# anihcsam/OpenGaussian

Measured on AMD Instinct MI355X. Metric: fwd+bwd Mpix/s at 1080p, 1M Gaussians (RGB+6-D ins_feat); k-means it/s, higher is better.
Workload: dtype f32; 1 GPU; S1M-1080p RGB(SH3)+depth+alpha (all grads) + 6-ch ins_feat (grad to ins_feat) fwd+bwd, ONE fused 9-channel pass; gaussians=1000000, width=1920, height=1080, views_cycled=8, parallelism=single

## Files before the change

opengaussian_amd/csrc/binning.hip:

```cpp
#include <stdlib.h>
#include <string.h>

#include "ogs_common.h"

namespace ogs {

namespace {

constexpr size_t kSweepHeaderWords = 4 * 256 + 4 + 60;
constexpr int kScanItems = 8;
constexpr int kScanTile = kBlock * kScanItems;

__device__ __forceinline__ uint32_t wave_inclusive_scan(uint32_t v) {
#pragma unroll
    for (int d = 1; d < kWave; d <<= 1) {
        uint32_t t = __shfl_up(v, d, kWave);
        if (lane_id() >= d) v += t;
    }
    return v;
}

__device__ __forceinline__ uint32_t block_exclusive_scan(uint32_t v, uint32_t& total, uint32_t* wave_sums ) {
    const int wave = threadIdx.x >> 6;
    const uint32_t inc = wave_inclusive_scan(v);
    if (lane_id() == kWave - 1) wave_sums[wave] = inc;
    __syncthreads();
    uint32_t base = 0, tot = 0;
#pragma unroll
    for (int w = 0; w < kBlock / kWave; ++w) {
        const uint32_t s = wave_sums[w];
        if (w < wave) base += s;
        tot += s;
    }
    total = tot;
    __syncthreads();
    return base + inc - v;
}

__device__ __forceinline__ void load_items(const uint32_t* __restrict__ in, const uint32_t* __restrict__ gather,
                                           int64_t base, int64_t n, uint32_t item[kScanItems]) {
#pragma unroll
    for (int i = 0; i < kScanItems; ++i) {
        const int64_t idx = base + i;
        uint32_t v = 0;
        if (idx < n) v = gather ? in[gather[idx]] : in[idx];
        item[i] = v;
    }
}

__global__ __launch_bounds__(kBlock) void scan_reduce_kernel(const uint32_t* __restrict__ in,
                                                             const uint32_t* __restrict__ gather, int64_t n,
                                                             uint32_t* __restrict__ partials, const uint32_t* __restrict__ n_dev) {
    __shared__ uint32_t wave_sums[4];
    if (n_dev) n = min(n, (int64_t)*n_dev);
    const int64_t base = (int64_t)blockIdx.x * kScanTile + (int64_t)threadIdx.x * kScanItems;
    uint32_t item[kScanItems];
    load_items(in, gather, base, n, item);
    uint32_t s = 0;
#pragma unroll
    for (int i = 0; i < kScanItems; ++i) s += item[i];
    uint32_t total;
    block_exclusive_scan(s, total, wave_sums);
    if (threadIdx.x == 0) partials[blockIdx.x] = total;
}

template <bool SUM_PARTIALS>
__global__ __launch_bounds__(kBlock) void scan_apply_kernel(const uint32_t* __restrict__ in,
                                                            const uint32_t* __restrict__ gather,
                                                            uint32_t* __restrict__ out, int64_t n,
                                                            const uint32_t* __restrict__ partial_offsets,
                                                            uint32_t* __restrict__ total_out, const uint32_t* __restrict__ n_dev) {
    __shared__ uint32_t wave_sums[4];
    if (n_dev) n = min(n, (int64_t)*n_dev);
    const int64_t base = (int64_t)blockIdx.x * kScanTile + (int64_t)threadIdx.x * kScanItems;
    uint32_t item[kScanItems];
    load_items(in, gather, base, n, item);
    uint32_t s = 0;
#pragma unroll
    for (int i = 0; i < kScanItems; ++i) s += item[i];
    uint32_t block_base = 0;
    if (SUM_PARTIALS) {
        uint32_t acc = 0;
        for (uint32_t j = threadIdx.x; j < blockIdx.x; j += kBlock) acc += partial_offsets[j];
        uint32_t tot;
        block_exclusive_scan(acc, tot, wave_sums);
        block_base = tot;
    } else if (partial_offsets) {
        block_base = partial_offsets[blockIdx.x];
    }
    uint32_t total;
    uint32_t run = block_exclusive_scan(s, total, wave_sums) + block_base;
#pragma unroll
    for (int i = 0; i < kScanItems; ++i) {
        const int64_t idx = base + i;
        if (idx < n) out[idx] = run;
        run += item[i];
    }
    if (total_out && threadIdx.x == 0) {
        if (SUM_PARTIALS) { if (blockIdx.x == gridDim.x - 1) *total_out = block_base + total; }
        else if (partial_offsets == nullptr) *total_out = total;
    }
}

__global__ void scan_total_kernel(const uint32_t* __restrict__ in, const uint32_t* __restrict__ gather,
                                  const uint32_t* __restrict__ out, int64_t n, uint32_t* __restrict__ total_out,
                                  const uint32_t* __restrict__ n_dev) {
    if (threadIdx.x == 0 && blockIdx.x == 0) {
        if (n_dev) n = min(n, (int64_t)*n_dev);
        if (n <= 0) { *total_out = 0u; return; }
        const uint32_t last = gather ? in[gather[n - 1]] : in[n - 1];
        *total_out = out[n - 1] + last;
    }
}

inline int scan_blocks(int64_t n) { return (int)((n + kScanTile - 1) / kScanTile); }
constexpr int kFlatScanBlocks = 16384;

template <int ITEMS>
__global__ __launch_bounds__(kBlock) void radix_hist_kernel(const uint32_t* __restrict__ keys, int64_t n_cap,
                                                            const uint32_t* __restrict__ n_dev, int shift,
                                                            int bits, uint32_t* __restrict__ hist, int nblocks, bool drop) {
    __shared__ uint32_t h[256];
    const int64_t n = n_dev ? min((int64_t)*n_dev, n_cap) : n_cap;
    const int ndig = 1 << bits;
    const uint32_t mask = ndig - 1;
    h[threadIdx.x] = 0;
    __syncthreads();
    const int64_t base = (int64_t)blockIdx.x * (kBlock * ITEMS);
#pragma unroll
    for (int i = 0; i < ITEMS; ++i) {
        const int64_t idx = base + i * kBlock + threadIdx.x;
        if (idx < n) {
            const uint32_t k = keys[idx];
            if (!(drop && k == kDropKey)) atomicAdd(&h[(k >> shift) & mask], 1u);
        }
    }
    __syncthreads();
    if ((int)threadIdx.x < ndig) hist[(size_t)threadIdx.x * nblocks + blockIdx.x] = h[threadIdx.x];
}

__global__ __launch_bounds__(kBlock) void radix_rowscan_kernel(uint32_t* __restrict__ hist, int nblocks,
                                                               uint32_t* __restrict__ row_total) {
    __shared__ uint32_t wave_sums[4];
    uint32_t* row = hist + (size_t)blockIdx.x * nblocks;
    uint32_t carry = 0;
    for (int base = 0; base < nblocks; base += kScanTile) {
        uint32_t item[kScanItems];
        const int b0 = base + (int)threadIdx.x * kScanItems;
        uint32_t sum = 0;
#pragma unroll
        for (int i = 0; i < kScanItems; ++i) {
            item[i] = (b0 + i < nblocks) ? row[b0 + i] : 0u;
            sum += item[i];
        }
        uint32_t total;
        uint32_t run = carry + block_exclusive_scan(sum, total, wave_sums);
#pragma unroll
        for (int i = 0; i < kScanItems; ++i) {
            if (b0 + i < nblocks) row[b0 + i] = run;
            run += item[i];
        }
        carry += total;
    }
    if (threadIdx.x == 0) row_total[blockIdx.x] = carry;
}

template <int ITEMS>
__global__ __launch_bounds__(kBlock) void radix_scatter_kernel(const uint32_t* __restrict__ keys_in,
                                                               const uint32_t* __restrict__ vals_in,
                                                               uint32_t* __restrict__ keys_out,
                                                               uint32_t* __restrict__ vals_out, int64_t n_cap,
                                                               const uint32_t* __restrict__ n_dev, int shift,
                                                               int bits, const uint32_t* __restrict__ offsets,
                                                               const uint32_t* __restrict__ row_total,
                                                               int nblocks, bool drop, uint32_t* __restrict__ kept_out) {
    __shared__ uint32_t wave_hist_s[kBlock / kWave][256];
    __shared__ uint32_t scan_sums[4];
    __shared__ uint32_t dig_start[256], glob_base[256];
    __shared__ uint32_t stage_k[kBlock * ITEMS], stage_v[kBlock * ITEMS];
    volatile uint32_t(*wave_hist)[256] = wave_hist_s;
    const int64_t n = n_dev ? min((int64_t)*n_dev, n_cap) : n_cap;
    const int ndig = 1 << bits;
    const uint32_t mask = ndig - 1;
    const int tid = threadIdx.x, lane = tid & 63, wave = tid >> 6;
#pragma unroll
    for (int w = 0; w < kBlock / kWave; ++w) wave_hist_s[w][tid] = 0;
    __syncthreads();

    const int64_t base = (int64_t)blockIdx.x * (kBlock * ITEMS) + (int64_t)wave * (ITEMS * kWave);
    uint32_t key[ITEMS], val[ITEMS], rank[ITEMS];
#pragma unroll
    for (int i = 0; i < ITEMS; ++i) {
        const int64_t idx = base + i * kWave + lane;
        const bool valid = idx < n;
        key[i] = valid ? keys_in[idx] : 0xFFFFFFFFu;
        val[i] = valid ? vals_in[idx] : 0u;
    }
    const uint64_t lt_mask = (1ull << lane) - 1ull;
#pragma unroll
    for (int i = 0; i < ITEMS; ++i) {
        const int64_t idx = base + i * kWave + lane;
        const bool valid = drop ? key[i] != kDropKey : idx < n;
        const uint32_t d = (key[i] >> shift) & mask;
        uint64_t peers = __ballot(valid);
        for (int b = 0; b < bits; ++b) {
            const bool bit = (d >> b) & 1u;
            const uint64_t m = __ballot(bit);
            peers &= bit ? m : ~m;
        }
        const uint32_t r = __popcll(peers & lt_mask);
        const uint32_t cnt = __popcll(peers);
        uint32_t pre = 0;
        if (valid) pre = wave_hist[wave][d];
        __builtin_amdgcn_wave_barrier();
        if (valid && r == 0) wave_hist[wave][d] = pre + cnt;
        __builtin_amdgcn_wave_barrier();
        rank[i] = pre + r;
    }
    __syncthreads();
    uint32_t run_len = 0;
    if (tid < ndig) {
#pragma unroll
        for (int w = 0; w < kBlock / kWave; ++w) {
            const uint32_t t = wave_hist_s[w][tid];
            wave_hist_s[w][tid] = run_len;
            run_len += t;
        }
    }
    uint32_t n_valid;
    const uint32_t local_start = block_exclusive_scan(run_len, n_valid, scan_sums);
    uint32_t dummy_total;
    const uint32_t digit_base = block_exclusive_scan(tid < ndig ? row_total[tid] : 0u, dummy_total, scan_sums);
    if (kept_out != nullptr && blockIdx.x == 0 && tid == 0) *kept_out = dummy_total;
    if (tid < ndig) {
        dig_start[tid] = local_start;
        glob_base[tid] = digit_base + offsets[(size_t)tid * nblocks + blockIdx.x] - local_start;
    }
    __syncthreads();
#pragma unroll
    for (int i = 0; i < ITEMS; ++i) {
        const int64_t idx = base + i * kWave + lane;
        if (drop ? key[i] != kDropKey : idx < n) {
            const uint32_t d = (key[i] >> shift) & mask;
            const uint32_t lp = dig_start[d] + wave_hist_s[wave][d] + rank[i];
            stage_k[lp] = key[i];
            stage_v[lp] = val[i];
        }
    }
    __syncthreads();
    for (uint32_t j = tid; j < n_valid; j += kBlock) {
        const uint32_t k = stage_k[j];
        const uint32_t pos = glob_base[(k >> shift) & mask] + j;
        keys_out[pos] = k;
        vals_out[pos] = stage_v[j];
    }
}

constexpr uint32_t kStatAgg = 1u << 30, kStatInc = 2u << 30, kStatMask = (1u << 30) - 1u;
constexpr int kSpinLimit = 1 << 22;
constexpr int kLookBack = 8;
constexpr int kHistAllBlocks = 256;

struct RadixPlanDev { int npass; int shift[4]; int bits[4]; };

__global__ __launch_bounds__(kBlock) void radix_hist_all_kernel(const uint32_t* __restrict__ keys, int64_t n_cap,
                                                                const uint32_t* __restrict__ n_dev, RadixPlanDev plan,
                                                                uint32_t* __restrict__ ghist , bool drop) {
    __shared__ uint32_t h[4][256];
    const int64_t n = n_dev ? min((int64_t)*n_dev, n_cap) : n_cap;
#pragma unroll
    for (int p = 0; p < 4; ++p) h[p][threadIdx.x] = 0;
    __syncthreads();
    for (int64_t idx = (int64_t)blockIdx.x * kBlock + threadIdx.x; idx < n; idx += (int64_t)gridDim.x * kBlock) {
        const uint32_t k = keys[idx];
        if (drop && k == kDropKey) continue;
#pragma unroll
        for (int p = 0; p < 4; ++p)
            if (p < plan.npass) atomicAdd(&h[p][(k >> plan.shift[p]) & ((1u << plan.bits[p]) - 1u)], 1u);
    }
    __syncthreads();
#pragma unroll
    for (int p = 0; p < 4; ++p)
        if (p < plan.npass && h[p][threadIdx.x] != 0) atomicAdd(&ghist[p * 256 + threadIdx.x], h[p][threadIdx.x]);
}

template <int ITEMS>
__global__ __launch_bounds__(kBlock) void radix_onesweep_kernel(const uint32_t* __restrict__ keys_in,
                                                                const uint32_t* __restrict__ vals_in,
                                                                uint32_t* __restrict__ keys_out,
                                                                uint32_t* __restrict__ vals_out, int64_t n_cap,
                                                                const uint32_t* __restrict__ n_dev, int shift, int bits,
                                                                const uint32_t* __restrict__ ghist ,
                                                                uint32_t* __restrict__ status ,
                                                                uint32_t* __restrict__ ticket ,
                                                                uint32_t* __restrict__ status_word ,
                                                                int spin_limit, bool drop,
                                                                uint32_t* __restrict__ kept_out) {
    __shared__ uint32_t wave_hist_s[kBlock / kWave][256];
    __shared__ uint32_t scan_sums[4];
    __shared__ uint32_t dig_start[256], glob_base[256];
    __shared__ uint32_t stage_k[kBlock * ITEMS], stage_v[kBlock * ITEMS];
    __shared__ uint32_t s_ticket;
    volatile uint32_t(*wave_hist)[256] = wave_hist_s;
    const int64_t n = n_dev ? min((int64_t)*n_dev, n_cap) : n_cap;
    const int ndig = 1 << bits;
    const uint32_t mask = ndig - 1;
    const int tid = threadIdx.x, lane = tid & 63, wave = tid >> 6;
    if (tid == 0) s_ticket = atomicAdd(ticket, 1u);
#pragma unroll
    for (int w = 0; w < kBlock / kWave; ++w) wave_hist_s[w][tid] = 0;
    __syncthreads();
    const uint32_t tile = s_ticket;
    if ((int64_t)tile * (kBlock * ITEMS) >= n) {
        if (kept_out != nullptr && tile == 0 && tid == 0) *kept_out = 0u;
        return;
    }

    const int64_t base = (int64_t)tile * (kBlock * ITEMS) + (int64_t)wave * (ITEMS * kWave);
    uint32_t key[ITEMS], val[ITEMS], rank[ITEMS];
#pragma unroll
    for (int i = 0; i < ITEMS; ++i) {
        const int64_t idx = base + i * kWave + lane;
        const bool valid = idx < n;
        key[i] = valid ? keys_in[idx] : 0xFFFFFFFFu;
        val[i] = valid ? vals_in[idx] : 0u;
    }
    const uint64_t lt_mask = (1ull << lane) - 1ull;
#pragma unroll
    for (int i = 0; i < ITEMS; ++i) {
        const int64_t idx = base + i * kWave + lane;
        const bool valid = drop ? key[i] != kDropKey : idx < n;
        const uint32_t d = (key[i] >> shift) & mask;
        uint64_t peers = __ballot(valid);
        for (int b = 0; b < bits; ++b) {
            const bool bit = (d >> b) & 1u;
            const uint64_t m = __ballot(bit);
            peers &= bit ? m : ~m;
        }
        const uint32_t r = __popcll(peers & lt_mask);
        const uint32_t cnt = __popcll(peers);
        uint32_t pre = 0;
        if (valid) pre = wave_hist[wave][d];
        __builtin_amdgcn_wave_barrier();
        if (valid && r == 0) wave_hist[wave][d] = pre + cnt;
        __builtin_amdgcn_wave_barrier();
        rank[i] = pre + r;
    }
    __syncthreads();
    uint32_t run_len = 0;
    if (tid < ndig) {
#pragma unroll
        for (int w = 0; w < kBlock / kWave; ++w) {
            const uint32_t t = wave_hist_s[w][tid];
            wave_hist_s[w][tid] = run_len;
            run_len += t;
        }
        __hip_atomic_store(&status[(size_t)tile * 256 + tid], (tile == 0 ? kStatInc : kStatAgg) | run_len,
                           __ATOMIC_RELAXED, __HIP_MEMORY_SCOPE_AGENT);
    }
    uint32_t n_valid;
    const uint32_t local_start = block_exclusive_scan(run_len, n_valid, scan_sums);
    uint32_t dummy_total;
    const uint32_t digit_base = block_exclusive_scan(tid < ndig ? ghist[tid] : 0u, dummy_total, scan_sums);
    if (kept_out != nullptr && tile == 0 && tid == 0) *kept_out = dummy_total;
    uint32_t before = 0;
    if (tid < ndig && tile > 0) {
        int64_t pb = (int64_t)tile - 1;
        int spins = 0;
        bool done = false;
        while (!done) {
            uint32_t sw[kLookBack];
#pragma unroll
            for (int k = 0; k < kLookBack; ++k)
                sw[k] = pb - k >= 0 ? __hip_atomic_load(&status[(size_t)(pb - k) * 256 + tid], __ATOMIC_RELAXED, __HIP_MEMORY_SCOPE_AGENT)
                                    : kStatInc;
            int used = 0;
#pragma unroll
            for (int k = 0; k < kLookBack; ++k) {
                if (done || used != k) continue;
                const uint32_t flag = sw[k] & ~kStatMask;
                if (flag == 0u) continue;
                before += sw[k] & kStatMask;
                used = k + 1;
                done = flag == kStatInc;
            }
            pb -= used;
            if (!done && used < kLookBack) {
                if (++spins > spin_limit) {
                    __hip_atomic_fetch_or(status_word, kAsyncRadixSpin, __ATOMIC_RELAXED, __HIP_MEMORY_SCOPE_SYSTEM);
                    break;
                }
                __builtin_amdgcn_s_sleep(1);
            }
        }
        __hip_atomic_store(&status[(size_t)tile * 256 + tid], kStatInc | ((before + run_len) & kStatMask),
                           __ATOMIC_RELAXED, __HIP_MEMORY_SCOPE_AGENT);
    }
    if (tid < ndig) {
        dig_start[tid] = local_start;
        glob_base[tid] = digit_base + before - local_start;
    }
    __syncthreads();
#pragma unroll
    for (int i = 0; i < ITEMS; ++i) {
        const int64_t idx = base + i * kWave + lane;
        if (drop ? key[i] != kDropKey : idx < n) {
            const uint32_t d = (key[i] >> shift) & mask;
            const uint32_t lp = dig_start[d] + wave_hist_s[wave][d] + rank[i];
            stage_k[lp] = key[i];
            stage_v[lp] = val[i];
        }
    }
    __syncthreads();
    for (uint32_t j = tid; j < n_valid; j += kBlock) {
        const uint32_t k = stage_k[j];
        const uint32_t pos = glob_base[(k >> shift) & mask] + j;
        if ((int64_t)pos < n) {
            keys_out[pos] = k;
            vals_out[pos] = stage_v[j];
        }
    }
}

constexpr int kRangeItems = 4;
__global__ __launch_bounds__(kBlock) void tile_ranges_kernel(const uint32_t* __restrict__ tile_keys, int64_t D_cap,
                                                             const uint32_t* __restrict__ n_dev,
                                                             uint2* __restrict__ ranges) {
    const int64_t D = n_dev ? min((int64_t)*n_dev, D_cap) : D_cap;
    const int64_t i0 = ((int64_t)blockIdx.x * kBlock + threadIdx.x) * kRangeItems;
    if (i0 >= D) return;
    uint32_t k[kRangeItems];
    if (i0 + kRangeItems <= D) {
        const uint4 v = *reinterpret_cast<const uint4*>(tile_keys + i0);
        k[0] = v.x; k[1] = v.y; k[2] = v.z; k[3] = v.w;
    } else {
#pragma unroll
        for (int j = 0; j < kRangeItems; ++j) k[j] = i0 + j < D ? tile_keys[i0 + j] : 0u;
    }
    uint32_t prev = i0 > 0 ? tile_keys[i0 - 1] : 0u;
#pragma unroll
    for (int j = 0; j < kRangeItems; ++j) {
        const int64_t i = i0 + j;
        if (i < D) {
            const uint32_t cur = k[j];
            if (i == 0) {
                ranges[cur].x = 0;
            } else if (prev != cur) {
                ranges[prev].y = (uint32_t)i;
                ranges[cur].x = (uint32_t)i;
            }
            if (i == D - 1) ranges[cur].y = (uint32_t)D;
            prev = cur;
        }
    }
}

constexpr int kTileSortWaves = kBlock / kWave;
struct TileSortLds {
    uint32_t hist[kTileSortWaves][256];
    uint32_t dig_start[256];
    uint32_t base[256];
    uint32_t scan_sums[4];
    uint32_t red[2];
    uint2 range[kTileSortWaves];
    uint32_t kv[2 * kTileSortCap];
};
typedef __attribute__((address_space(3))) volatile uint32_t LdsWord;
typedef __attribute__((address_space(3))) unsigned long long LdsMask;
__device__ __forceinline__ LdsWord* lds_words(uint32_t* p) { return (LdsWord*)p; }
__device__ __forceinline__ LdsMask* wave_masks(TileSortLds& sm, int wave) { return (LdsMask*)(sm.kv + wave * 2 * kWaveSortCap); }

__device__ __forceinline__ void wave_rank_clear(LdsWord* hist, LdsMask* masks) {
    const int lane = threadIdx.x & (kWave - 1);
#pragma unroll
    for (int j = 0; j < 4; ++j) {
        hist[lane + j * kWave] = 0u;
        __hip_atomic_store(&masks[lane + j * kWave], 0ull, __ATOMIC_SEQ_CST, __HIP_MEMORY_SCOPE_WAVEFRONT);
    }
    __builtin_amdgcn_wave_barrier();
}

__device__ __forceinline__ void wave_rank(LdsWord* hist, LdsMask* masks, const uint32_t (&key)[kTileSortItems],
                                          uint32_t (&rank)[kTileSortItems], int ipl, int first, int m, int shift,
                                          uint32_t mask) {
    const int lane = threadIdx.x & (kWave - 1);
    const unsigned long long me = 1ull << lane;
#pragma unroll
    for (int i = 0; i < kTileSortItems; ++i) {
        if (i >= ipl) continue;
        const bool valid = first + i * kWave + lane < m;
        const uint32_t d = (key[i] >> shift) & mask;
        if (valid) __hip_atomic_fetch_or(&masks[d], me, __ATOMIC_SEQ_CST, __HIP_MEMORY_SCOPE_WAVEFRONT);
        __builtin_amdgcn_wave_barrier();
        const unsigned long long peers =
            valid ? __hip_atomic_load(&masks[d], __ATOMIC_SEQ_CST, __HIP_MEMORY_SCOPE_WAVEFRONT) : 0ull;
        const uint32_t r = __builtin_amdgcn_mbcnt_hi((uint32_t)(peers >> 32), __builtin_amdgcn_mbcnt_lo((uint32_t)peers, 0u));
        uint32_t pre = 0;
        if (valid) pre = hist[d];
        __builtin_amdgcn_wave_barrier();
        if (valid && r == 0) {
            hist[d] = pre + (uint32_t)__popcll(peers);
            __hip_atomic_store(&masks[d], 0ull, __ATOMIC_SEQ_CST, __HIP_MEMORY_SCOPE_WAVEFRONT);
        }
        __builtin_amdgcn_wave_barrier();
        rank[i] = pre + r;
    }
}

__device__ __forceinline__ void load_items(const uint32_t* __restrict__ list, const uint32_t* __restrict__ depth_keys,
                                           uint32_t (&key)[kTileSortItems], uint32_t (&val)[kTileSortItems], int ipl, int first,
                                           int m) {
#pragma unroll
    for (int i = 0; i < kTileSortItems; ++i) {
        if (i >= ipl) continue;
        val[i] = list[min(first + i * kWave, m - 1)];
    }
#pragma unroll
    for (int i = 0; i < kTileSortItems; ++i) {
        if (i >= ipl) continue;
        key[i] = depth_keys[val[i] & kGidMask];
    }
}

__device__ __forceinline__ uint32_t tile_sort_rank(TileSortLds& sm, const uint32_t (&key)[kTileSortItems],
                                                   uint32_t (&rank)[kTileSortItems], int ipl, int chunk, int m, int shift,
                                                   uint32_t mask) {
    const int tid = threadIdx.x, wave = tid >> 6;
    LdsWord* hist = lds_words(sm.hist[wave]);
    LdsMask* masks = wave_masks(sm, wave);
    wave_rank_clear(hist, masks);
    wave_rank(hist, masks, key, rank, ipl, wave * chunk, m, shift, mask);
    __syncthreads();
    uint32_t run_len = 0;
#pragma unroll
    for (int w = 0; w < kTileSortWaves; ++w) {
        const uint32_t t = sm.hist[w][tid];
        sm.hist[w][tid] = run_len;
        run_len += t;
    }
    uint32_t total;
    sm.dig_start[tid] = block_exclusive_scan(run_len, total, sm.scan_sums);
    __syncthreads();
    return run_len;
}

__device__ __forceinline__ void wave_sort_list(TileSortLds& sm, uint32_t* __restrict__ seg, int n,
                                               const uint32_t* __restrict__ depth_keys) {
    const int lane = threadIdx.x & (kWave - 1), wave = threadIdx.x >> 6;
    LdsWord* wk = lds_words(sm.kv + wave * 2 * kWaveSortCap);
    LdsWord* wv = wk + kWaveSortCap;
    LdsWord* hist = lds_words(sm.hist[wave]);
    LdsMask* masks = wave_masks(sm, wave);
    uint32_t key[kTileSortItems], val[kTileSortItems], rank[kTileSortItems];
    const int ipl = (n + kWave - 1) / kWave;
    load_items(seg, depth_keys, key, val, ipl, lane, n);
    uint32_t k_and = 0xFFFFFFFFu, k_or = 0u;
#pragma unroll
    for (int i = 0; i < kTileSortItems; ++i) {
        if (i >= ipl) continue;
        k_and &= key[i];
        k_or |= key[i];
    }
#pragma unroll
    for (int d = 32; d >= 1; d >>= 1) {
        k_and &= (uint32_t)__shfl_xor((int)k_and, d, kWave);
        k_or |= (uint32_t)__shfl_xor((int)k_or, d, kWave);
    }
    const uint32_t diff = (uint32_t)__builtin_amdgcn_readfirstlane((int)(k_and ^ k_or));
    if (diff == 0u) return;
    const int lo = __builtin_ctz(diff), hi = 31 - __builtin_clz(diff);
    const int npass = (hi - lo + 8) / 8;
    const int per = (hi - lo + npass) / npass;
    for (int p = 0; p < npass; ++p) {
        const int shift = lo + p * per, bits = min(per, hi + 1 - shift);
        const uint32_t mask = (1u << bits) - 1u;
        wave_rank_clear(hist, masks);
        wave_rank(hist, masks, key, rank, ipl, 0, n, shift, mask);
        uint32_t c[4], sum = 0;
#pragma unroll
        for (int j = 0; j < 4; ++j) { c[j] = hist[4 * lane + j]; sum += c[j]; }
        uint32_t run = wave_inclusive_scan(sum) - sum;
#pragma unroll
        for (int j = 0; j < 4; ++j) { hist[4 * lane + j] = run; run += c[j]; }
        __builtin_amdgcn_wave_barrier();
#pragma unroll
        for (int i = 0; i < kTileSortItems; ++i) {
            if (i >= ipl) continue;
            rank[i] += hist[(key[i] >> shift) & mask];
        }
#pragma unroll
        for (int i = 0; i < kTileSortItems; ++i) {
            if (i >= ipl) continue;
            if (i * kWave + lane < n) {
                wk[rank[i]] = key[i];
                wv[rank[i]] = val[i];
            }
        }
        __builtin_amdgcn_wave_barrier();
        if (p + 1 < npass) {
#pragma unroll
            for (int i = 0; i < kTileSortItems; ++i) {
                if (i >= ipl) continue;
                const int e = min(i * kWave + lane, n - 1);
                key[i] = wk[e];
                val[i] = wv[e];
            }
            __builtin_amdgcn_wave_barrier();
        }
    }
    for (int j = lane; j < n; j += kWave) seg[j] = wv[j];
}

__device__ __forceinline__ void block_sort_list(TileSortLds& sm, uint32_t* __restrict__ seg, uint32_t* __restrict__ alt, int n,
                                                const uint32_t* __restrict__ depth_keys) {
    const int tid = threadIdx.x, lane = tid & 63, wave = tid >> 6;
    const bool in_lds = n <= kTileSortCap;
    uint32_t key[kTileSortItems], val[kTileSortItems], rank[kTileSortItems];
    __syncthreads();
    if (tid < 2) sm.red[tid] = tid == 0 ? 0xFFFFFFFFu : 0u;
    uint32_t k_and = 0xFFFFFFFFu, k_or = 0u;
    const int ipl0 = (min(n, kTileSortCap) + kBlock - 1) / kBlock, chunk0 = ipl0 * kWave;
    if (in_lds) {
        load_items(seg, depth_keys, key, val, ipl0, wave * chunk0 + lane, n);
#pragma unroll
        for (int i = 0; i < kTileSortItems; ++i) {
            if (i >= ipl0) continue;
            k_and &= key[i];
            k_or |= key[i];
        }
    } else {
        for (int j = tid; j < n; j += kBlock) {
            const uint32_t k = depth_keys[seg[j] & kGidMask];
            k_and &= k;
            k_or |= k;
        }
    }
#pragma unroll
    for (int d = 32; d >= 1; d >>= 1) {
        k_and &= (uint32_t)__shfl_xor((int)k_and, d, kWave);
        k_or |= (uint32_t)__shfl_xor((int)k_or, d, kWave);
    }
    __syncthreads();
    if (lane == 0) { atomicAnd(&sm.red[0], k_and); atomicOr(&sm.red[1], k_or); }
    __syncthreads();
    const uint32_t diff = sm.red[0] ^ sm.red[1];
    if (diff == 0u) return;
    const int lo = __builtin_ctz(diff), hi = 31 - __builtin_clz(diff);
    const int npass = (hi - lo + 8) / 8;
    const int per = (hi - lo + npass) / npass;
    uint32_t* const sk = sm.kv;
    uint32_t* const sv = sm.kv + kTileSortCap;

    if (in_lds) {
        for (int p = 0; p < npass; ++p) {
            const int shift = lo + p * per, bits = min(per, hi + 1 - shift);
            const uint32_t mask = (1u << bits) - 1u;
            tile_sort_rank(sm, key, rank, ipl0, chunk0, n, shift, mask);
#pragma unroll
            for (int i = 0; i < kTileSortItems; ++i) {
                if (i >= ipl0) continue;
                const uint32_t d = (key[i] >> shift) & mask;
                rank[i] += sm.dig_start[d] + sm.hist[wave][d];
            }
#pragma unroll
            for (int i = 0; i < kTileSortItems; ++i) {
                if (i >= ipl0) continue;
                if (wave * chunk0 + i * kWave + lane < n) {
                    sk[rank[i]] = key[i];
                    sv[rank[i]] = val[i];
                }
            }
            __syncthreads();
            if (p + 1 < npass) {
#pragma unroll
                for (int i = 0; i < kTileSortItems; ++i) {
                    if (i >= ipl0) continue;
                    const int e = min(wave * chunk0 + i * kWave + lane, n - 1);
                    key[i] = sk[e];
                    val[i] = sv[e];
                }
                __syncthreads();
            }
        }
        for (int j = tid; j < n; j += kBlock) seg[j] = sv[j];
        return;
    }

    for (int p = 0; p < npass; ++p) {
        const int shift = lo + p * per, bits = min(per, hi + 1 - shift);
        const uint32_t mask = (1u << bits) - 1u;
        const uint32_t* __restrict__ src = (p & 1) ? alt : seg;
        uint32_t* __restrict__ dst = (p & 1) ? seg : alt;
        sm.base[tid] = 0u;
        __syncthreads();
        for (int j = tid; j < n; j += kBlock) atomicAdd(&sm.base[(depth_keys[src[j] & kGidMask] >> shift) & mask], 1u);
        __syncthreads();
        uint32_t total;
        const uint32_t start = block_exclusive_scan(sm.base[tid], total, sm.scan_sums);
        sm.base[tid] = start;
        for (int c0 = 0; c0 < n; c0 += kTileSortCap) {
            const int m = min(kTileSortCap, n - c0);
            const int ipl = (m + kBlock - 1) / kBlock, chunk = ipl * kWave;
            load_items(src + c0, depth_keys, key, val, ipl, wave * chunk + lane, m);
            const uint32_t cnt = tile_sort_rank(sm, key, rank, ipl, chunk, m, shift, mask);
#pragma unroll
            for (int i = 0; i < kTileSortItems; ++i) {
                if (i >= ipl) continue;
                if (wave * chunk + i * kWave + lane < m) {
                    const uint32_t d = (key[i] >> shift) & mask;
                    dst[sm.base[d] + sm.hist[wave][d] + rank[i]] = val[i];
                }
            }
            __syncthreads();
            sm.base[tid] += cnt;
        }
        __syncthreads();
    }
    if (npass & 1) {
        for (int j = tid; j < n; j += kBlock) seg[j] = alt[j];
    }
}

__global__ __launch_bounds__(kBlock) void tile_depth_sort_kernel(const uint2* __restrict__ ranges, int tiles,
                                                                 const uint32_t* __restrict__ tile_order,
                                                                 uint32_t* __restrict__ point_list,
                                                                 const uint32_t* __restrict__ depth_keys,
                                                                 uint32_t* __restrict__ scratch) {
    __shared__ TileSortLds sm;
    const int wave = threadIdx.x >> 6;
    if (threadIdx.x < kTileSortWaves) {
        const int b = blockIdx.x * kTileSortWaves + threadIdx.x;
        sm.range[threadIdx.x] = b < tiles ? ranges[tile_order ? tile_order[b] : (uint32_t)b] : make_uint2(0u, 0u);
    }
    __syncthreads();
    const uint32_t x = (uint32_t)__builtin_amdgcn_readfirstlane((int)sm.range[wave].x);
    const int n = __builtin_amdgcn_readfirstlane((int)(sm.range[wave].y - sm.range[wave].x));
    if (n >= 2 && n <= kWaveSortCap) wave_sort_list(sm, point_list + x, n, depth_keys);
#pragma unroll 1
    for (int w = 0; w < kTileSortWaves; ++w) {
        const uint32_t xw = (uint32_t)__builtin_amdgcn_readfirstlane((int)sm.range[w].x);
        const int nw = __builtin_amdgcn_readfirstlane((int)(sm.range[w].y - sm.range[w].x));
        if (nw > kWaveSortCap) block_sort_list(sm, point_list + xw, scratch + xw, nw, depth_keys);
    }
}

__global__ __launch_bounds__(kBlock) void export_keys_kernel(const uint2* __restrict__ ranges,
                                                             const uint32_t* __restrict__ point_list,
                                                             const float4* __restrict__ rec, int recv4,
                                                             uint64_t* __restrict__ keys_out) {
    const uint32_t tile = blockIdx.x;
    const uint2 r = ranges[tile];
    for (uint32_t i = r.x + threadIdx.x; i < r.y; i += kBlock) {
        const uint32_t gid = point_list[i] & kGidMask;
        const uint32_t bits = __float_as_uint(rec[(size_t)gid * recv4].z);
        keys_out[i] = ((uint64_t)tile << 32) | bits;
    }
}

}

size_t scan_tmp_bytes(int64_t n) {
    size_t total = 0;
    int64_t m = n;
    while (true) {
        const int nb = scan_blocks(m);
        if (nb <= 1) break;
        total += align_up((size_t)nb * sizeof(uint32_t));
        m = nb;
    }
    return total + kAlign;
}

size_t sort_tmp_bytes(int64_t n) {
    const int64_t hist = (int64_t)256 * sort_blocks_for(n > 0 ? n : 1);
    const size_t legacy = align_up((size_t)hist * sizeof(uint32_t)) + align_up(256 * sizeof(uint32_t)) + scan_tmp_bytes(hist);
    const int64_t tiles4 = ((n > 0 ? n : 1) + kBlock * 4 - 1) / (kBlock * 4);
    const size_t sweep = align_up(kSweepHeaderWords * sizeof(uint32_t)) + 4 * align_up((size_t)256 * tiles4 * sizeof(uint32_t));
    return legacy > sweep ? legacy : sweep;
}

static int sweep_items_for(int64_t n, int forced) {
    if (forced == 4 || forced == 16) return forced;
    return n <= (int64_t)(256 << 10) ? 4 : 16;
}

bool radix_onesweep_enabled(int64_t n) {
    static const int forced = [] {
        const char* e = getenv("OGS_RADIX");
        return !e ? 0 : strcmp(e, "legacy") == 0 ? 1 : strcmp(e, "sweep") == 0 ? 2 : 0;
    }();
    if (forced == 1 || n >= (int64_t)kStatMask) return false;
    return forced == 2 || n <= (int64_t)(256 << 10);
}

namespace {
struct SweepTmp {
    uint32_t* ghist;
    uint32_t* ticket;
    uint32_t* status[4];
    size_t zero_bytes;
    static SweepTmp carve(void* tmp, int64_t n, int npass, int items_forced) {
        SweepTmp t;
        char* p = static_cast<char*>(tmp);
        t.ghist = reinterpret_cast<uint32_t*>(p);
        t.ticket = t.ghist + 4 * 256;
        const int items = sweep_items_for(n, items_forced);
        const int64_t tiles = ((n > 0 ? n : 1) + (int64_t)kBlock * items - 1) / ((int64_t)kBlock * items);
        const size_t table = align_up((size_t)256 * tiles * sizeof(uint32_t));
        char* q = p + align_up(kSweepHeaderWords * sizeof(uint32_t));
        for (int i = 0; i < 4; ++i) t.status[i] = reinterpret_cast<uint32_t*>(q + (size_t)i * table);
        t.zero_bytes = align_up(kSweepHeaderWords * sizeof(uint32_t)) + (size_t)npass * table;
        return t;
    }
};
}

int radix_sort_begin(const uint32_t* keys, int64_t n, const uint32_t* n_dev, int npass, const int* shifts, const int* bits,
                     void* tmp, hipStream_t stream, int debug, bool drop, int items) {
    if (n <= 0) return OGS_OK;
    if (npass < 1 || npass > 4) { set_error("radix_sort_begin: npass=%d out of range", npass); return OGS_ERR_INVALID_ARG; }
    const SweepTmp t = SweepTmp::carve(tmp, n, npass, items);
    OGS_HIP_CHECK(hipMemsetAsync(tmp, 0, t.zero_bytes, stream));
    RadixPlanDev plan{};
    plan.npass = npass;
    for (int i = 0; i < npass; ++i) {
        if (bits[i] < 1 || bits[i] > 8) { set_error("radix_sort_begin: bits=%d out of range", bits[i]); return OGS_ERR_INVALID_ARG; }
        plan.shift[i] = shifts[i];
        plan.bits[i] = bits[i];
    }
    const int64_t want = (n + kBlock * 16 - 1) / (kBlock * 16);
    const int grid = (int)(want < 1 ? 1 : (want > kHistAllBlocks ? kHistAllBlocks : want));
    OGS_LAUNCH(radix_hist_all_kernel, dim3(grid), dim3(kBlock), 0, stream, keys, n, n_dev, plan, t.ghist, drop);
    OGS_LAUNCH_CHECK(debug, stream);
    return OGS_OK;
}

int radix_sort_pass(int pass, int npass, const uint32_t* keys_in, const uint32_t* vals_in, uint32_t* keys_out, uint32_t* vals_out,
                    int64_t n, int shift, int bits, void* tmp, hipStream_t stream, int debug, const uint32_t* n_dev, bool drop,
                    uint32_t* kept_out, int items_forced, int spin_limit) {
    if (n <= 0) return OGS_OK;
    const SweepTmp t = SweepTmp::carve(tmp, n, npass, items_forced);
    const int items = sweep_items_for(n, items_forced);
    const int nb = (int)((n + (int64_t)kBlock * items - 1) / ((int64_t)kBlock * items));
    uint32_t* status_word = async_status_word();
    if (!status_word) return OGS_ERR_HIP;
    if (spin_limit < 0) spin_limit = kSpinLimit;
    if (items == 4) {
        OGS_LAUNCH(radix_onesweep_kernel<4>, dim3(nb), dim3(kBlock), 0, stream, keys_in, vals_in, keys_out, vals_out, n, n_dev,
                   shift, bits, (const uint32_t*)(t.ghist + pass * 256), t.status[pass], t.ticket + pass, status_word, spin_limit,
                   drop, kept_out);
    } else {
        OGS_LAUNCH(radix_onesweep_kernel<16>, dim3(nb), dim3(kBlock), 0, stream, keys_in, vals_in, keys_out, vals_out, n, n_dev,
                   shift, bits, (const uint32_t*)(t.ghist + pass * 256), t.status[pass], t.ticket + pass, status_word, spin_limit,
                   drop, kept_out);
    }
    OGS_LAUNCH_CHECK(debug, stream);
    return OGS_OK;
}

int exclusive_scan_u32(const uint32_t* in, const uint32_t* gather, uint32_t* out, int64_t n, uint32_t* total,
                       void* tmp, hipStream_t stream, int debug, const uint32_t* n_dev) {
    if (n <= 0) {
        if (total) OGS_HIP_CHECK(hipMemsetAsync(total, 0, sizeof(uint32_t), stream));
        return OGS_OK;
    }
    const int nb = scan_blocks(n);
    if (nb == 1) {
        OGS_LAUNCH(scan_apply_kernel<false>, dim3(1), dim3(kBlock), 0, stream, in, gather, out, n,
                           (const uint32_t*)nullptr, total, n_dev);
        OGS_LAUNCH_CHECK(debug, stream);
        return OGS_OK;
    }
    uint32_t* partials = static_cast<uint32_t*>(tmp);
    void* next_tmp = static_cast<char*>(tmp) + align_up((size_t)nb * sizeof(uint32_t));
    OGS_LAUNCH(scan_reduce_kernel, dim3(nb), dim3(kBlock), 0, stream, in, gather, n, partials, n_dev);
    OGS_LAUNCH_CHECK(debug, stream);
    if (nb <= kFlatScanBlocks) {
        OGS_LAUNCH(scan_apply_kernel<true>, dim3(nb), dim3(kBlock), 0, stream, in, gather, out, n,
                           (const uint32_t*)partials, total, n_dev);
        OGS_LAUNCH_CHECK(debug, stream);
        return OGS_OK;
    }
    int rc = exclusive_scan_u32(partials, nullptr, partials, nb, nullptr, next_tmp, stream, debug, nullptr);
    if (rc != OGS_OK) return rc;
    OGS_LAUNCH(scan_apply_kernel<false>, dim3(nb), dim3(kBlock), 0, stream, in, gather, out, n,
                       (const uint32_t*)partials, (uint32_t*)nullptr, n_dev);
    OGS_LAUNCH_CHECK(debug, stream);
    if (total) {
        if (in == out) { set_error("exclusive_scan_u32: total with in-place scan unsupported"); return OGS_ERR_INVALID_ARG; }
        OGS_LAUNCH(scan_total_kernel, dim3(1), dim3(64), 0, stream, in, gather, (const uint32_t*)out, n, total, n_dev);
        OGS_LAUNCH_CHECK(debug, stream);
    }
    return OGS_OK;
}

int radix_pass(const uint32_t* keys_in, const uint32_t* vals_in, uint32_t* keys_out, uint32_t* vals_out, int64_t n,
               int shift, int bits, void* tmp, hipStream_t stream, int debug, const uint32_t* n_dev, bool drop,
               uint32_t* kept_out) {
    if (n <= 0) return OGS_OK;
    if (bits < 1 || bits > 8) { set_error("radix_pass: bits=%d out of range", bits); return OGS_ERR_INVALID_ARG; }
    const int items = sort_items_for(n);
    const int nb = sort_blocks_for(n);
    const int ndig = 1 << bits;
    uint32_t* hist = static_cast<uint32_t*>(tmp);
    uint32_t* row_total = reinterpret_cast<uint32_t*>(static_cast<char*>(tmp) + align_up((size_t)256 * nb * sizeof(uint32_t)));
    if (items == 4) {
        OGS_LAUNCH(radix_hist_kernel<4>, dim3(nb), dim3(kBlock), 0, stream, keys_in, n, n_dev, shift, bits, hist, nb, drop);
    } else {
        OGS_LAUNCH(radix_hist_kernel<8>, dim3(nb), dim3(kBlock), 0, stream, keys_in, n, n_dev, shift, bits, hist, nb, drop);
    }
    OGS_LAUNCH_CHECK(debug, stream);
    OGS_LAUNCH(radix_rowscan_kernel, dim3(ndig), dim3(kBlock), 0, stream, hist, nb, row_total);
    OGS_LAUNCH_CHECK(debug, stream);
    if (items == 4) {
        OGS_LAUNCH(radix_scatter_kernel<4>, dim3(nb), dim3(kBlock), 0, stream, keys_in, vals_in, keys_out, vals_out, n, n_dev,
                   shift, bits, (const uint32_t*)hist, (const uint32_t*)row_total, nb, drop, kept_out);
    } else {
        OGS_LAUNCH(radix_scatter_kernel<8>, dim3(nb), dim3(kBlock), 0, stream, keys_in, vals_in, keys_out, vals_out, n, n_dev,
                   shift, bits, (const uint32_t*)hist, (const uint32_t*)row_total, nb, drop, kept_out);
    }
    OGS_LAUNCH_CHECK(debug, stream);
    return OGS_OK;
}

int launch_tile_ranges(const uint32_t* tile_keys_sorted, int64_t D, uint2* ranges, int64_t tiles, hipStream_t s,
                       int debug, const uint32_t* n_dev, bool already_zeroed) {
    if (!already_zeroed) OGS_HIP_CHECK(hipMemsetAsync(ranges, 0, (size_t)tiles * sizeof(uint2), s));
    if (D <= 0) return OGS_OK;
    const int grid = (int)((D + (int64_t)kBlock * kRangeItems - 1) / ((int64_t)kBlock * kRangeItems));
    OGS_LAUNCH(tile_ranges_kernel, dim3(grid), dim3(kBlock), 0, s, tile_keys_sorted, D, n_dev, ranges);
    OGS_LAUNCH_CHECK(debug, s);
    return OGS_OK;
}

int launch_tile_depth_sort(const uint2* ranges, int64_t tiles, const uint32_t* tile_order, uint32_t* point_list,
                           const uint32_t* depth_keys, uint32_t* scratch, hipStream_t s, int debug) {
    if (tiles <= 0) return OGS_OK;
    if (tiles >= (1ll << 31)) { set_error("tile_depth_sort: %lld tiles", (long long)tiles); return OGS_ERR_UNSUPPORTED; }
    const unsigned grid = (unsigned)((tiles + kTileSortWaves - 1) / kTileSortWaves);
    OGS_LAUNCH(tile_depth_sort_kernel, dim3(grid), dim3(kBlock), 0, s, ranges, (int)tiles, tile_order, point_list, depth_keys,
               scratch);
    OGS_LAUNCH_CHECK(debug, s);
    return OGS_OK;
}

int launch_export_keys(const uint2* ranges, int tiles, const uint32_t* point_list, const float4* rec, int recv4,
                       uint64_t* keys_out, hipStream_t s) {
    OGS_LAUNCH(export_keys_kernel, dim3(tiles), dim3(kBlock), 0, s, ranges, point_list, rec, recv4, keys_out);
    OGS_LAUNCH_CHECK(0, s);
    return OGS_OK;
}

}
```

Before: 1452 Mpix/s.

## Batch wave radix ranking with LDS peer-mask tables across several items

Replaces the per-bit ballot match loop in the global radix scatter/onesweep kernels with a shared LDS peer-mask ranking routine that handles several items per batch. Each batch's per-digit masks live in the staging buffer, and a per-digit walk assigns running offsets, so fewer wave barriers and atomics are needed per item. The per-tile and per-wave sorts now use the same batched routine with a relaxed fetch_or. The intent is to cut ballot and LDS-round-trip latency during binning sorts. In exchange it adds LDS traffic for mask clearing and scanning all digits for each batch, and it depends on subtle wavefront memory ordering.

Result: no change. 1442 Mpix/s (-0.6%).

```diff
diff --git a/opengaussian_amd/csrc/binning.hip b/opengaussian_amd/csrc/binning.hip
--- a/opengaussian_amd/csrc/binning.hip
+++ b/opengaussian_amd/csrc/binning.hip
@@ -116,6 +116,131 @@
 inline int scan_blocks(int64_t n) { return (int)((n + kScanTile - 1) / kScanTile); }
 constexpr int kFlatScanBlocks = 16384;
 
+typedef __attribute__((address_space(3))) volatile uint32_t LdsWord;
+typedef __attribute__((address_space(3))) volatile unsigned long long LdsMask;
+__device__ __forceinline__ LdsWord* lds_words(uint32_t* p) { return (LdsWord*)p; }
+constexpr int kRankBatch = 4;
+constexpr int kBlockRankBatch = 2;
+
+__device__ __forceinline__ void rank_step() {
+    __builtin_amdgcn_fence(__ATOMIC_SEQ_CST, "wavefront");
+    __builtin_amdgcn_wave_barrier();
+}
+
+template <int K, int STRIDE>
+__device__ __forceinline__ void wave_masks_clear(LdsMask* masks, int ndig) {
+    const int lane = threadIdx.x & (kWave - 1);
+#pragma unroll
+    for (int j = 0; j < 4; ++j) {
+        if (j * kWave >= ndig) continue;
+#pragma unroll
+        for (int k = 0; k < K; ++k) masks[k * STRIDE + j * kWave + lane] = 0ull;
+    }
+    rank_step();
+}
+
+template <int K, int STRIDE, int R>
+__device__ __forceinline__ void wave_rank_batch(LdsWord* hist, LdsMask* masks, int ndig, int live, const uint32_t (&d)[K],
+                                                const bool (&valid)[K], uint32_t (&rank)[K]) {
+    const int lane = threadIdx.x & (kWave - 1);
+    const unsigned long long me = 1ull << lane;
+#pragma unroll
+    for (int k = 0; k < K; ++k) {
+        if (k >= live) continue;
+        if (valid[k]) __hip_atomic_fetch_or(&masks[k * STRIDE + d[k]], me, __ATOMIC_RELAXED, __HIP_MEMORY_SCOPE_WAVEFRONT);
+    }
+    rank_step();
+    unsigned long long peers[K];
+#pragma unroll
+    for (int k = 0; k < K; ++k) {
+        if (k >= live) continue;
+        peers[k] = masks[k * STRIDE + d[k]];
+    }
+#pragma unroll
+    for (int j0 = 0; j0 < 4; j0 += R) {
+        if (j0 * kWave >= ndig) continue;
+        unsigned long long own[R][K];
+        uint32_t run[R];
+#pragma unroll
+        for (int j = 0; j < R; ++j) {
+            if ((j0 + j) * kWave >= ndig) continue;
+            const int dg = min((j0 + j) * kWave + lane, ndig - 1);
+            run[j] = hist[dg];
+#pragma unroll
+            for (int k = 0; k < K; ++k) {
+                if (k >= live) continue;
+                own[j][k] = masks[k * STRIDE + dg];
+            }
+        }
+        rank_step();
+#pragma unroll
+        for (int j = 0; j < R; ++j) {
+            if ((j0 + j) * kWave >= ndig) continue;
+            const int dg = (j0 + j) * kWave + lane;
+            if (dg < ndig) {
+                uint32_t r = run[j];
+#pragma unroll
+                for (int k = 0; k < K; ++k) {
+                    if (k >= live) continue;
+                    if (own[j][k] != 0ull) *(LdsWord*)&masks[k * STRIDE + dg] = r;
+                    r += (uint32_t)__popcll(own[j][k]);
+                }
+                if (r != run[j]) hist[dg] = r;
+            }
+        }
+        rank_step();
+    }
+#pragma unroll
+    for (int k = 0; k < K; ++k) {
+        if (k >= live) continue;
+        const uint32_t before = *(LdsWord*)&masks[k * STRIDE + d[k]];
+        rank[k] = valid[k] ? before : 0u;
+    }
+    rank_step();
+#pragma unroll
+    for (int k = 0; k < K; ++k) {
+        if (k >= live) continue;
+        const unsigned long long p = valid[k] ? peers[k] : 0ull;
+        const uint32_t r = __builtin_amdgcn_mbcnt_hi((uint32_t)(p >> 32), __builtin_amdgcn_mbcnt_lo((uint32_t)p, 0u));
+        if (valid[k] && r == 0u) masks[k * STRIDE + d[k]] = 0ull;
+        rank[k] += r;
+    }
+    rank_step();
+}
+
+template <int ITEMS, int K, int STRIDE>
+__device__ __forceinline__ void radix_rank_items(LdsWord* hist, LdsMask* masks, int ndig, const uint32_t (&key)[ITEMS],
+                                                 uint32_t (&rank)[ITEMS], int64_t first, int64_t n, int shift, bool drop) {
+    static_assert(ITEMS % K == 0, "whole batches");
+    const int lane = threadIdx.x & (kWave - 1);
+    wave_masks_clear<K, STRIDE>(masks, ndig);
+#pragma unroll
+    for (int b = 0; b < ITEMS; b += K) {
+        uint32_t d[K], r[K];
+        bool valid[K];
+#pragma unroll
+        for (int k = 0; k < K; ++k) {
+            d[k] = (key[b + k] >> shift) & (uint32_t)(ndig - 1);
+            valid[k] = drop ? key[b + k] != kDropKey : first + (b + k) * kWave + lane < n;
+        }
+        wave_rank_batch<K, STRIDE, 2>(hist, masks, ndig, K, d, valid, r);
+#pragma unroll
+        for (int k = 0; k < K; ++k) rank[b + k] = r[k];
+    }
+}
+
+template <int ITEMS>
+__device__ __forceinline__ void radix_rank_wave(LdsWord* hist, uint32_t* stage, int ndig, const uint32_t (&key)[ITEMS],
+                                                uint32_t (&rank)[ITEMS], int64_t first, int64_t n, int shift, bool drop) {
+    constexpr int kMasks = kWave * ITEMS, kWide = ITEMS >= 4 * kRankBatch ? kRankBatch : (ITEMS >= 4 ? ITEMS / 4 : 1);
+    static_assert(kWide * 256 <= kMasks, "a wave's masks fit its share of the staging space");
+    LdsMask* masks = (LdsMask*)stage + (threadIdx.x >> 6) * kMasks;
+    if (kRankBatch * ndig <= kMasks)
+        radix_rank_items<ITEMS, kRankBatch, kMasks / kRankBatch>(hist, masks, ndig, key, rank, first, n, shift, drop);
+    else
+        radix_rank_items<ITEMS, kWide, 256>(hist, masks, ndig, key, rank, first, n, shift, drop);
+}
+
 template <int ITEMS>
 __global__ __launch_bounds__(kBlock) void radix_hist_kernel(const uint32_t* __restrict__ keys, int64_t n_cap,
                                                             const uint32_t* __restrict__ n_dev, int shift,
@@ -177,8 +302,9 @@
     __shared__ uint32_t wave_hist_s[kBlock / kWave][256];
     __shared__ uint32_t scan_sums[4];
     __shared__ uint32_t dig_start[256], glob_base[256];
-    __shared__ uint32_t stage_k[kBlock * ITEMS], stage_v[kBlock * ITEMS];
-    volatile uint32_t(*wave_hist)[256] = wave_hist_s;
+    __shared__ __attribute__((aligned(16))) uint32_t stage[2 * kBlock * ITEMS];
+    uint32_t* const stage_k = stage;
+    uint32_t* const stage_v = stage + kBlock * ITEMS;
     const int64_t n = n_dev ? min((int64_t)*n_dev, n_cap) : n_cap;
     const int ndig = 1 << bits;
     const uint32_t mask = ndig - 1;
@@ -196,27 +322,7 @@
         key[i] = valid ? keys_in[idx] : 0xFFFFFFFFu;
         val[i] = valid ? vals_in[idx] : 0u;
     }
-    const uint64_t lt_mask = (1ull << lane) - 1ull;
-#pragma unroll
-    for (int i = 0; i < ITEMS; ++i) {
-        const int64_t idx = base + i * kWave + lane;
-        const bool valid = drop ? key[i] != kDropKey : idx < n;
-        const uint32_t d = (key[i] >> shift) & mask;
-        uint64_t peers = __ballot(valid);
-        for (int b = 0; b < bits; ++b) {
-            const bool bit = (d >> b) & 1u;
-            const uint64_t m = __ballot(bit);
-            peers &= bit ? m : ~m;
-        }
-        const uint32_t r = __popcll(peers & lt_mask);
-        const uint32_t cnt = __popcll(peers);
-        uint32_t pre = 0;
-        if (valid) pre = wave_hist[wave][d];
-        __builtin_amdgcn_wave_barrier();
-        if (valid && r == 0) wave_hist[wave][d] = pre + cnt;
-        __builtin_amdgcn_wave_barrier();
-        rank[i] = pre + r;
-    }
+    radix_rank_wave<ITEMS>(lds_words(wave_hist_s[wave]), stage, ndig, key, rank, base, n, shift, drop);
     __syncthreads();
     uint32_t run_len = 0;
     if (tid < ndig) {
@@ -299,9 +405,10 @@
     __shared__ uint32_t wave_hist_s[kBlock / kWave][256];
     __shared__ uint32_t scan_sums[4];
     __shared__ uint32_t dig_start[256], glob_base[256];
-    __shared__ uint32_t stage_k[kBlock * ITEMS], stage_v[kBlock * ITEMS];
+    __shared__ __attribute__((aligned(16))) uint32_t stage[2 * kBlock * ITEMS];
+    uint32_t* const stage_k = stage;
+    uint32_t* const stage_v = stage + kBlock * ITEMS;
     __shared__ uint32_t s_ticket;
-    volatile uint32_t(*wave_hist)[256] = wave_hist_s;
     const int64_t n = n_dev ? min((int64_t)*n_dev, n_cap) : n_cap;
     const int ndig = 1 << bits;
     const uint32_t mask = ndig - 1;
@@ -325,27 +432,7 @@
         key[i] = valid ? keys_in[idx] : 0xFFFFFFFFu;
         val[i] = valid ? vals_in[idx] : 0u;
     }
-    const uint64_t lt_mask = (1ull << lane) - 1ull;
-#pragma unroll
-    for (int i = 0; i < ITEMS; ++i) {
-        const int64_t idx = base + i * kWave + lane;
-        const bool valid = drop ? key[i] != kDropKey : idx < n;
-        const uint32_t d = (key[i] >> shift) & mask;
-        uint64_t peers = __ballot(valid);
-        for (int b = 0; b < bits; ++b) {
-            const bool bit = (d >> b) & 1u;
-            const uint64_t m = __ballot(bit);
-            peers &= bit ? m : ~m;
-        }
-        const uint32_t r = __popcll(peers & lt_mask);
-        const uint32_t cnt = __popcll(peers);
-        uint32_t pre = 0;
-        if (valid) pre = wave_hist[wave][d];
-        __builtin_amdgcn_wave_barrier();
-        if (valid && r == 0) wave_hist[wave][d] = pre + cnt;
-        __builtin_amdgcn_wave_barrier();
-        rank[i] = pre + r;
-    }
+    radix_rank_wave<ITEMS>(lds_words(wave_hist_s[wave]), stage, ndig, key, rank, base, n, shift, drop);
     __syncthreads();
     uint32_t run_len = 0;
     if (tid < ndig) {
@@ -465,45 +552,35 @@
     uint2 range[kTileSortWaves];
     uint32_t kv[2 * kTileSortCap];
 };
-typedef __attribute__((address_space(3))) volatile uint32_t LdsWord;
-typedef __attribute__((address_space(3))) unsigned long long LdsMask;
-__device__ __forceinline__ LdsWord* lds_words(uint32_t* p) { return (LdsWord*)p; }
 __device__ __forceinline__ LdsMask* wave_masks(TileSortLds& sm, int wave) { return (LdsMask*)(sm.kv + wave * 2 * kWaveSortCap); }
 
-__device__ __forceinline__ void wave_rank_clear(LdsWord* hist, LdsMask* masks) {
+__device__ __forceinline__ void wave_rank_clear(LdsWord* hist, LdsMask* masks, int ndig) {
     const int lane = threadIdx.x & (kWave - 1);
 #pragma unroll
-    for (int j = 0; j < 4; ++j) {
-        hist[lane + j * kWave] = 0u;
-        __hip_atomic_store(&masks[lane + j * kWave], 0ull, __ATOMIC_SEQ_CST, __HIP_MEMORY_SCOPE_WAVEFRONT);
-    }
-    __builtin_amdgcn_wave_barrier();
-}
-
+    for (int j = 0; j < 4; ++j) hist[lane + j * kWave] = 0u;
+    wave_masks_clear<kRankBatch, 256>(masks, ndig);
+}
+
+template <int K, int R>
 __device__ __forceinline__ void wave_rank(LdsWord* hist, LdsMask* masks, const uint32_t (&key)[kTileSortItems],
                                           uint32_t (&rank)[kTileSortItems], int ipl, int first, int m, int shift,
                                           uint32_t mask) {
+    static_assert(kTileSortItems % K == 0 && K * 256 * 8 <= 2 * kWaveSortCap * 4,
+                  "the tables of a batch fit a wave's quarter of the key / value space");
     const int lane = threadIdx.x & (kWave - 1);
-    const unsigned long long me = 1ull << lane;
-#pragma unroll
-    for (int i = 0; i < kTileSortItems; ++i) {
-        if (i >= ipl) continue;
-        const bool valid = first + i * kWave + lane < m;
-        const uint32_t d = (key[i] >> shift) & mask;
-        if (valid) __hip_atomic_fetch_or(&masks[d], me, __ATOMIC_SEQ_CST, __HIP_MEMORY_SCOPE_WAVEFRONT);
-        __builtin_amdgcn_wave_barrier();
-        const unsigned long long peers =
-            valid ? __hip_atomic_load(&masks[d], __ATOMIC_SEQ_CST, __HIP_MEMORY_SCOPE_WAVEFRONT) : 0ull;
-        const uint32_t r = __builtin_amdgcn_mbcnt_hi((uint32_t)(peers >> 32), __builtin_amdgcn_mbcnt_lo((uint32_t)peers, 0u));
-        uint32_t pre = 0;
-        if (valid) pre = hist[d];
-        __builtin_amdgcn_wave_barrier();
-        if (valid && r == 0) {
-            hist[d] = pre + (uint32_t)__popcll(peers);
-            __hip_atomic_store(&masks[d], 0ull, __ATOMIC_SEQ_CST, __HIP_MEMORY_SCOPE_WAVEFRONT);
-        }
-        __builtin_amdgcn_wave_barrier();
-        rank[i] = pre + r;
+#pragma unroll
+    for (int b = 0; b < kTileSortItems; b += K) {
+        if (b >= ipl) continue;
+        uint32_t d[K], r[K];
+        bool valid[K];
+#pragma unroll
+        for (int k = 0; k < K; ++k) {
+            d[k] = (key[b + k] >> shift) & mask;
+            valid[k] = first + (b + k) * kWave + lane < m;
+        }
+        wave_rank_batch<K, 256, R>(hist, masks, (int)mask + 1, min(K, ipl - b), d, valid, r);
+#pragma unroll
+        for (int k = 0; k < K; ++k) rank[b + k] = r[k];
     }
 }
 
@@ -528,8 +605,8 @@
     const int tid = threadIdx.x, wave = tid >> 6;
     LdsWord* hist = lds_words(sm.hist[wave]);
     LdsMask* masks = wave_masks(sm, wave);
-    wave_rank_clear(hist, masks);
-    wave_rank(hist, masks, key, rank, ipl, wave * chunk, m, shift, mask);
+    wave_rank_clear(hist, masks, (int)mask + 1);
+    wave_rank<kBlockRankBatch, 1>(hist, masks, key, rank, ipl, wave * chunk, m, shift, mask);
     __syncthreads();
     uint32_t run_len = 0;
 #pragma unroll
@@ -574,8 +651,8 @@
     for (int p = 0; p < npass; ++p) {
         const int shift = lo + p * per, bits = min(per, hi + 1 - shift);
         const uint32_t mask = (1u << bits) - 1u;
-        wave_rank_clear(hist, masks);
-        wave_rank(hist, masks, key, rank, ipl, 0, n, shift, mask);
+        wave_rank_clear(hist, masks, (int)mask + 1);
+        wave_rank<kRankBatch, 2>(hist, masks, key, rank, ipl, 0, n, shift, mask);
         uint32_t c[4], sum = 0;
 #pragma unroll
         for (int j = 0; j < 4; ++j) { c[j] = hist[4 * lane + j]; sum += c[j]; }
```
